# FeatureBaseDB/featurebase

Measured on NVIDIA H100. Metric: set_ops_per_sec, higher is better.
Workload: dtype u64/u16 integer

## Files before the change

### featurebase_b200/csrc/fbgpu.cu

```cuda
#include <cuda_runtime.h>
#include <dlfcn.h>
#include <fcntl.h>
#include <sys/mman.h>
#include <sys/stat.h>
#include <unistd.h>
#include <stdarg.h>
#include <stdio.h>
#include <string.h>

#include <algorithm>
#include <condition_variable>
#include <map>
#include <memory>
#include <mutex>
#include <shared_mutex>
#include <atomic>
#include <deque>
#include <functional>
#include <string>
#include <thread>
#include <unordered_map>
#include <vector>

#include "../../include/fbgpu.h"
// ... 793 lines not shown
    c->meta_dirty = true; c->tables_valid = false; c->dev_tables_valid = false;
    return commit_locked(c);
}

extern "C" int fbgpu_commit(fbgpu_ctx* c) try {
    if (!c) return fail(FBGPU_E_INVALID, "null ctx");
    std::unique_lock<std::shared_mutex> lk(c->store_mu);
    if (!c->inspect_only && c->dead_arena >= (256ull << 20) && c->dead_arena * 2 >= c->uploaded + c->staging.len) return compact_locked(c);
    return commit_locked(c);
} FBGPU_CATCH

extern "C" int fbgpu_compact(fbgpu_ctx* c) try {
    if (!c) return fail(FBGPU_E_INVALID, "null ctx");
    std::unique_lock<std::shared_mutex> lk(c->store_mu);
    return compact_locked(c);
} FBGPU_CATCH
static int lock_committed(fbgpu_ctx* c, std::shared_lock<std::shared_mutex>& lk) {
    if (c->inspect_only) return fail(FBGPU_E_CUDA, "this context was created with FBGPU_DEVICE_NONE: it holds no device and answers no query");
    for (;;) {
        lk = std::shared_lock<std::shared_mutex>(c->store_mu);
        if (!c->meta_dirty && c->staging.empty()) return 0;
        lk.unlock();
        int rc = fbgpu_commit(c); if (rc) return rc;
    }
}

extern "C" int fbgpu_get_stats(fbgpu_ctx* c, fbgpu_stats* out) try {
    if (!c || !out) return fail(FBGPU_E_INVALID, "null argument");
    std::shared_lock<std::shared_mutex> lk(c->store_mu);
    *out = c->stats;
    return 0;
} FBGPU_CATCH

static int compile_program(fbgpu_ctx* c, uint32_t index, const fbgpu_op* ops, int32_t n_ops, std::vector<DevOp>& out, int& depth) {
    Error err;
    ViewLookup lookup = [c, index](uint32_t field, uint32_t view) { return view_id_locked(c, ViewKey{ index, field, view }, false); };
    int rc = compile(ops, n_ops, lookup, out, depth, err);
    if (rc) return fail(rc, "%s", err.msg);
#ifndef FBGPU_WP_LEGACY_LOOP
    expand_push_row(out);
#endif
    return 0;
}

static void bump(fbgpu_ctx* c, uint64_t launches, float ms) {
    std::lock_guard<std::mutex> lk(c->cnt_mu);
    c->counters.kernel_launches += launches; c->counters.queries++; c->counters.last_query_gpu_ms = ms;
}

static int allreduce_u64(fbgpu_ctx* c, Workspace* w, void* dptr, size_t n) {
    if (!c->comm) return 0;
    std::lock_guard<std::mutex> lk(c->coll_mu);
    int r = g_nccl.AllReduce(dptr, dptr, n, kNcclUint64, kNcclSum, c->comm, w->stream);
    if (r != 0) return fail(FBGPU_E_COMM, "ncclAllReduce failed: %s", g_nccl.GetErrorString ? g_nccl.GetErrorString(r) : "?");
    return 0;
}

static std::vector<int2> find_batches(const std::vector<DevOp>& prog);
static int upload_inputs(Workspace* w, const std::vector<DevOp>& prog, const uint64_t* shards, int64_t n_shards, const DevOp** d_prog, const uint64_t** d_shards) {
    std::vector<int2> batches = find_batches(prog);
    size_t pb = prog.size() * sizeof(DevOp), sb = (size_t)n_shards * 8, bb = batches.size() * sizeof(int2), tot = pb + sb + bb;
    if (w->h_in.ensure(tot + 16)) return FBGPU_E_NOMEM;
    if (w->d_in.ensure(pb + sb + 16)) return FBGPU_E_NOMEM;
    if (w->d_aux.ensure(bb + 16)) return FBGPU_E_NOMEM;
    if (pb) memcpy(w->h_in.p, prog.data(), pb);
    if (sb) memcpy((uint8_t*)w->h_in.p + pb, shards, sb);
    if (bb) memcpy((uint8_t*)w->h_in.p + pb + sb, batches.data(), bb);
    if (pb + sb) CUDA_TRY(cudaMemcpyAsync(w->d_in.p, w->h_in.p, pb + sb, cudaMemcpyHostToDevice, w->stream));
    if (bb) CUDA_TRY(cudaMemcpyAsync(w->d_aux.p, (uint8_t*)w->h_in.p + pb + sb, bb, cudaMemcpyHostToDevice, w->stream));
    *d_prog = (const DevOp*)w->d_in.p; *d_shards = (const uint64_t*)((uint8_t*)w->d_in.p + pb);
    return 0;
}

static std::vector<int2> find_batches(const std::vector<DevOp>& prog) {
    std::vector<int2> b;
    for (size_t k = 0; k < prog.size();) {
        uint8_t o = prog[k].op;
        if (o == D_OR_ROW || o == D_ANDNOT_ROW || o == D_XOR_ROW) { size_t e = k + 1; while (e < prog.size() && prog[e].op == o) e++; b.push_back(make_int2((int)k, (int)e)); k = e; }
        else k++;
    }
    return b;
}

static int launch_eval(fbgpu_ctx* c, Workspace* w, const std::vector<DevOp>& prog, const DevOp* d_prog, int depth, const uint64_t* d_shards, long long n_units, EvalOut out) {
    if (n_units <= 0) return 0;
    const int n_ops = (int)prog.size();
    std::vector<int2> batches = find_batches(prog);
    size_t staged_rows = 0; for (auto& b : batches) staged_rows += (size_t)(b.y - b.x);
    if (!out.info && n_ops <= kWpMaxOps && depth <= kWpMaxDepth && !getenv("FBGPU_NO_WORDPAR")) {
        uint64_t arr = 0, other = 0, striped = 0;
        for (const DevOp& o : prog) if (o.op >= D_PUSH_ROW && o.op <= D_ORANDNOT_ROW && o.op != D_PUSH_EMPTY && o.fv < c->view_arr.size()) { arr += c->view_arr[o.fv]; other += c->view_other[o.fv]; striped += c->view_striped[o.fv]; }
        if (striped == 0 && ((other > 0 && arr * 8 <= other) || getenv("FBGPU_FORCE_WORDPAR") != nullptr)) {
            long long blocks = n_units * kWpBlocksPerUnit;
            long long grid = std::min<long long>(blocks, (long long)c->sm_count * std::max(FBGPU_WP_MIN_BLOCKS, 8) * 2);
            eval_wordpar_kernel<<<(unsigned)grid, kWpThreads, 0, w->stream>>>(store_ref(c), d_prog, n_ops, d_shards, n_units, out);
            CUDA_TRY(cudaGetLastError());
            return 0;
        }
    }
    const bool staged = getenv("FBGPU_STAGED") && n_ops <= kStagedMaxOps && staged_rows >= 4;
    const int2* d_batches = reinterpret_cast<const int2*>(w->d_aux.p);
    if (staged) {
        int ctas = 2;
        if (const char* e = getenv("FBGPU_STAGE_CTAS")) ctas = std::max(1, std::min(4, atoi(e)));
        const size_t per_cta = 233472 / ctas - 1024 - 5888;
        size_t stack = (size_t)(depth + 1) * 8192;
        if (stack + 2 * 8192 <= per_cta) {
            uint32_t stg = (uint32_t)(((per_cta - stack) / 2) & ~size_t(127));
            long long grid = std::min<long long>(n_units, (long long)c->sm_count * ctas);
            size_t smem = stack + 2 * (size_t)stg;
            eval_staged_kernel<<<(unsigned)grid, kEvalThreads, smem, w->stream>>>(store_ref(c), d_prog, n_ops, depth, d_batches, (int)batches.size(), stg, d_shards, n_units, out);
            CUDA_TRY(cudaGetLastError());
            return 0;
        }
    }
    size_t smem = (size_t)(depth + 1) * 8192;
    int per_sm = std::max(1, (int)std::min<size_t>(std::min(FBGPU_EVAL_MIN_BLOCKS, 2048 / kEvalThreads), (227 * 1024) / (smem + 3 * 1024 + 512)));
    long long grid = std::min<long long>(n_units, (long long)c->sm_count * per_sm);
    eval_kernel<<<(unsigned)grid, kEvalThreads, smem, w->stream>>>(store_ref(c), d_prog, n_ops, depth, d_batches, (int)batches.size(), d_shards, n_units, out);
    CUDA_TRY(cudaGetLastError());
    return 0;
}

static bool contiguous_shards(const uint64_t* shards, int64_t n) {
    for (int64_t i = 1; i < n; i++) if (shards[i] != shards[0] + (uint64_t)i) return false;
    return n > 0;
}

static int count_impl(fbgpu_ctx* c, uint32_t index, const fbgpu_op* ops, int32_t n_ops, const uint64_t* shards, int64_t n_shards,
                      uint64_t* out_total, uint64_t* out_per_shard, bool collective) {
    if (!c || !out_total || n_shards < 0 || (n_shards && !shards)) return fail(FBGPU_E_INVALID, "null argument");
    USE_DEVICE(c);
    std::shared_lock<std::shared_mutex> lk;
    int rc = lock_committed(c, lk); if (rc) return rc;
    std::vector<DevOp> prog; int depth = 1;
    rc = compile_program(c, index, ops, n_ops, prog, depth); if (rc) return rc;
    WsLease lease(c); Workspace* w = lease.w;
    const DevOp* d_prog; const uint64_t* d_shards;
    rc = upload_inputs(w, prog, shards, n_shards, &d_prog, &d_shards); if (rc) return rc;
    const size_t nper = out_per_shard ? (size_t)n_shards : 0, nc = 1 + nper + 3;
    if (w->d_counts.ensure(nc * 8)) return FBGPU_E_NOMEM;
    if (w->h_out.ensure(nc * 8)) return FBGPU_E_NOMEM;
    CUDA_TRY(cudaMemsetAsync(w->d_counts.p, 0, nc * 8, w->stream));
    unsigned long long* d_total = (unsigned long long*)w->d_counts.p;
    unsigned long long* d_per = out_per_shard ? d_total + 1 : nullptr;
    long long n_units = (long long)n_shards * kSlotsPerRow;
    std::unique_lock<std::mutex> coll_lk(c->coll_mu, std::defer_lock);
    FuseReduce fr{};
    coll_lk.lock();
    const bool p2p = c->p2p && collective;
    if (!p2p) coll_lk.unlock();
    if (p2p) {
        fr.peers = (Mailbox* const*)c->d_peers.p; fr.ticket = (unsigned int*)(d_total + 1 + nper); fr.result = d_total + 1 + nper + 1;
        fr.error = (unsigned int*)(d_total + 1 + nper + 2);
        fr.epoch = ++c->epoch; fr.rank = c->rank; fr.n_ranks = c->n_ranks; fr.timeout_cycles = c->p2p_timeout_cycles;
    }
    CUDA_TRY(cudaEventRecord(w->ev0, w->stream));
    if (n_units > 0) {
        const DevOp* pa = nullptr; const DevOp* pb = nullptr;
        if (prog.size() == 2 && prog[0].op == D_PUSH_ROW && prog[1].op == D_AND_ROW) { pa = &prog[0]; pb = &prog[1]; }
        else if (prog.size() == 3 && prog[0].op == D_PUSH_EMPTY && prog[1].op == D_OR_ROW && prog[2].op == D_AND_ROW) { pa = &prog[1]; pb = &prog[2]; }
        if (pa && !getenv("FBGPU_NO_PAIR_KERNEL")) {
            long long grid = std::min<long long>((n_units + kPcWarps - 1) / kPcWarps, (long long)c->sm_count * c->pair_ctas_per_sm);
            c->counters_pair_launches++;
            pair_count_kernel<<<(unsigned)grid, kPcWarps * 32, kPcWarps * 8192, w->stream>>>(store_ref(c), pa->fv, pa->row, pb->fv, pb->row, nullptr, nullptr, n_units,
                contiguous_shards(shards, n_shards) ? nullptr : d_shards, n_shards ? shards[0] : 0, n_units, d_total, d_per, nullptr, fr);
            CUDA_TRY(cudaGetLastError());
        } else {
            EvalOut eo{ d_total, d_per, nullptr, nullptr, fr };
            rc = launch_eval(c, w, prog, d_prog, depth, d_shards, n_units, eo); if (rc) return rc;
        }
    } else if (p2p) {
        p2p_reduce_only_kernel<<<1, 1, 0, w->stream>>>(fr, d_total);
        CUDA_TRY(cudaGetLastError());
    }
    if (!p2p && collective) { rc = allreduce_u64(c, w, d_total, 1); if (rc) return rc; }
    CUDA_TRY(cudaEventRecord(w->ev1, w->stream));
    CUDA_TRY(cudaMemcpyAsync(w->h_out.p, w->d_counts.p, nc * 8, cudaMemcpyDeviceToHost, w->stream));
    CUDA_TRY(cudaStreamSynchronize(w->stream));
    if (p2p && ((uint64_t*)w->h_out.p)[1 + nper + 2] != 0) {
        lease.ok = true;
        return fail(FBGPU_E_COMM, "rank %d did not publish its count for exchange %llu in time (peer dead, or the ranks issued their collective queries in different orders); re-open with fbgpu_comm_p2p_open",
                    (int)((uint64_t*)w->h_out.p)[1 + nper + 2] - 1, (unsigned long long)fr.epoch);
    }
    *out_total = p2p ? ((uint64_t*)w->h_out.p)[1 + nper + 1] : ((uint64_t*)w->h_out.p)[0];
    if (out_per_shard) memcpy(out_per_shard, (uint64_t*)w->h_out.p + 1, (size_t)n_shards * 8);
    float ms = 0; cudaEventElapsedTime(&ms, w->ev0, w->ev1);
    bump(c, (n_units > 0 || p2p) ? 1 : 0, ms);
    lease.ok = true;
    return FBGPU_OK;
}
extern "C" int fbgpu_count(fbgpu_ctx* c, uint32_t index, const fbgpu_op* ops, int32_t n_ops, const uint64_t* shards, int64_t n_shards,
                           uint64_t* out_total, uint64_t* out_per_shard) try {
    return count_impl(c, index, ops, n_ops, shards, n_shards, out_total, out_per_shard, true);
} FBGPU_CATCH
static int fbgpu_count_local(fbgpu_ctx* c, uint32_t index, const fbgpu_op* ops, int32_t n_ops, const uint64_t* shards, int64_t n_shards, uint64_t* out_total) {
    return count_impl(c, index, ops, n_ops, shards, n_shards, out_total, nullptr, false);
}

extern "C" int fbgpu_row(fbgpu_ctx* c, uint32_t index, const fbgpu_op* ops, int32_t n_ops, const uint64_t* shards, int64_t n_shards,
                         uint8_t* out_buf, uint64_t out_cap, uint64_t* out_len, uint64_t* out_count) try {
    if (!c || !out_len || n_shards < 0 || (n_shards && !shards)) return fail(FBGPU_E_INVALID, "null argument");
    USE_DEVICE(c);
    std::shared_lock<std::shared_mutex> lk;
    int rc = lock_committed(c, lk); if (rc) return rc;
    std::vector<DevOp> prog; int depth = 1;
    rc = compile_program(c, index, ops, n_ops, prog, depth); if (rc) return rc;
    std::vector<uint64_t> sorted(shards, shards + n_shards);
    std::sort(sorted.begin(), sorted.end());
    sorted.erase(std::unique(sorted.begin(), sorted.end()), sorted.end());
    n_shards = (int64_t)sorted.size();
    WsLease lease(c); Workspace* w = lease.w;
    const DevOp* d_prog; const uint64_t* d_shards;
    rc = upload_inputs(w, prog, sorted.data(), n_shards, &d_prog, &d_shards); if (rc) return rc;
    long long n_units = (long long)n_shards * kSlotsPerRow;
    struct OutCont { uint64_t key; uint16_t typ; uint32_t n; uint64_t size; uint32_t batch; uint64_t src_off; };
    std::vector<OutCont> conts; std::vector<std::vector<uint8_t>> batch_bufs;
    const bool single_batch = n_units <= c->unit_batch;
    const uint8_t* single_src = nullptr;
    uint64_t total_count = 0; uint64_t launches = 0; float ms_total = 0;
    for (long long u0 = 0; u0 < n_units; u0 += c->unit_batch) {
        long long nu = std::min(c->unit_batch, n_units - u0);
        if (w->d_bitmaps.ensure((size_t)nu * 8192)) return FBGPU_E_NOMEM;
        if (w->d_info.ensure((size_t)nu * 8)) return FBGPU_E_NOMEM;
        if (w->h_out.ensure((size_t)nu * 8)) return FBGPU_E_NOMEM;
        EvalOut eo{ nullptr, nullptr, (uint4*)w->d_bitmaps.p, (uint2*)w->d_info.p, FuseReduce{} };
        CUDA_TRY(cudaEventRecord(w->ev0, w->stream));
        rc = launch_eval(c, w, prog, d_prog, depth, d_shards + u0 / kSlotsPerRow, nu, eo); if (rc) return rc;
        launches++;
        CUDA_TRY(cudaMemcpyAsync(w->h_out.p, w->d_info.p, (size_t)nu * 8, cudaMemcpyDeviceToHost, w->stream));
        CUDA_TRY(cudaStreamSynchronize(w->stream));
        std::vector<EmitUnit> emits; uint64_t off = 0; size_t first = conts.size();
        const uint2* info = (const uint2*)w->h_out.p;
        for (long long u = 0; u < nu; u++) {
            uint32_t N = info[u].x, runs = info[u].y;
            if (!N) continue;
            uint16_t typ = (runs <= 2048 && runs <= N / 2) ? kRun : (N < 4096 ? kArray : kBitmap);
            uint64_t size = typ == kRun ? 2 + 4ull * runs : typ == kArray ? 2ull * N : 8192;
            EmitUnit e{ off, (uint32_t)u, typ };
            emits.push_back(e);
            OutCont oc; oc.key = sorted[(u0 + u) / kSlotsPerRow] * kSlotsPerRow + (uint64_t)((u0 + u) % kSlotsPerRow); oc.typ = typ; oc.n = N; oc.size = size;
            oc.batch = (uint32_t)batch_bufs.size(); oc.src_off = off;
            conts.push_back(oc);
            off += (size + 15) & ~15ull;
            total_count += N;
        }
        if (emits.empty()) batch_bufs.emplace_back();
        if (!emits.empty()) {
            if (w->d_emit_units.ensure(emits.size() * sizeof(EmitUnit))) return FBGPU_E_NOMEM;
// ... 707 lines not shown
```

### featurebase_b200/csrc/kernels.cuh

```cuda
#pragma once
#include <cuda_runtime.h>
#include <stdint.h>
#include "fbgpu_types.h"
#include "bitaddr.h"
#include "wp_machine.h"
#include "resolve.h"

namespace fbgpu {

#ifndef FBGPU_EVAL_THREADS
#define FBGPU_EVAL_THREADS 256
#endif
#ifndef FBGPU_EVAL_MIN_BLOCKS
#define FBGPU_EVAL_MIN_BLOCKS 6
#endif
constexpr int kEvalThreads = FBGPU_EVAL_THREADS;
constexpr int kEvalU4PerThread = 512 / kEvalThreads;
constexpr int kEvalW64PerThread = 1024 / kEvalThreads;
constexpr int kResolveChunk = 128;

__device__ __forceinline__ uint4 ldg_nc(const uint4* p) {
    uint4 r;
    asm volatile("ld.global.nc.L1::no_allocate.v4.u32 {%0,%1,%2,%3}, [%4];" : "=r"(r.x), "=r"(r.y), "=r"(r.z), "=r"(r.w) : "l"(p));
    return r;
// ... 71 lines not shown
    for (int h = 0; h < kEvalU4PerThread; h++) {
        int i = threadIdx.x + h * kEvalThreads;
        uint4 x = ldg_nc(g + i);
        switch (kind) {
            case K_PUSH: top[i] = x; break;
            case K_OR: top[i] = or4(top[i], x); break;
            case K_AND: top[i] = and4(top[i], x); break;
            case K_ANDNOT: top[i] = andn4(top[i], x); break;
            case K_XOR: top[i] = xor4(top[i], x); break;
            case K_ORAND: below[i] = or4(below[i], and4(top[i], x)); break;
            default: below[i] = or4(below[i], andn4(top[i], x)); break;
        }
    }
}
__device__ __forceinline__ void bm_apply_smem(int kind, uint4* top, uint4* below, const uint4* s) {
#pragma unroll
    for (int h = 0; h < kEvalU4PerThread; h++) {
        int i = threadIdx.x + h * kEvalThreads;
        uint4 x = s[i];
        switch (kind) {
            case K_PUSH: top[i] = x; break;
            case K_OR: top[i] = or4(top[i], x); break;
            case K_AND: top[i] = and4(top[i], x); break;
            case K_ANDNOT: top[i] = andn4(top[i], x); break;
            case K_XOR: top[i] = xor4(top[i], x); break;
            case K_ORAND: below[i] = or4(below[i], and4(top[i], x)); break;
            default: below[i] = or4(below[i], andn4(top[i], x)); break;
        }
    }
}

template <int MODE>
__device__ __forceinline__ void smem_bit_op(uint32_t* bm, uint32_t v) {
    uint32_t addr = (uint32_t)__cvta_generic_to_shared(bm + (v >> 5));
    uint32_t m = 1u << (v & 31);
    if (MODE == 0) asm volatile("red.shared.or.b32 [%0], %1;" :: "r"(addr), "r"(m) : "memory");
    else if (MODE == 1) asm volatile("red.shared.and.b32 [%0], %1;" :: "r"(addr), "r"(~m) : "memory");
    else asm volatile("red.shared.xor.b32 [%0], %1;" :: "r"(addr), "r"(m) : "memory");
}
template <int MODE>
__device__ __forceinline__ void warp_bitmap_atomic(uint32_t* bm, const uint4* g, int lane) {
    for (int i = lane; i < 512; i += 32) {
        uint4 v = ldg_nc(g + i);
        uint32_t w[4] = { v.x, v.y, v.z, v.w };
#pragma unroll
        for (int q = 0; q < 4; q++) {
            if (MODE == 0) atomicOr(&bm[4 * i + q], w[q]); else if (MODE == 1) atomicAnd(&bm[4 * i + q], ~w[q]); else atomicXor(&bm[4 * i + q], w[q]);
        }
    }
}
template <int MODE>
__device__ __forceinline__ void smem_bit_op_at(uint32_t addr, uint32_t sh) {
    const uint32_t m = 1u << (sh & 31);
    if (MODE == 0) asm volatile("red.shared.or.b32 [%0], %1;" :: "r"(addr), "r"(m) : "memory");
    else if (MODE == 1) asm volatile("red.shared.and.b32 [%0], %1;" :: "r"(addr), "r"(~m) : "memory");
    else asm volatile("red.shared.xor.b32 [%0], %1;" :: "r"(addr), "r"(m) : "memory");
}
template <int MODE>
__device__ __forceinline__ void scatter_chunk_sb(smem_base_t sb, uint4 v, uint32_t base, uint32_t n) {
    uint32_t w[4] = { v.x, v.y, v.z, v.w };
    if (MODE != 2 || base + 8 <= n) {
#pragma unroll
        for (int q = 0; q < 4; q++) {
            smem_bit_op_at<MODE>(word_addr_lo(sb, w[q]), w[q]);
            smem_bit_op_at<MODE>(word_addr_hi(sb, w[q]), upper16(w[q]));
        }
    } else {
#pragma unroll
        for (int q = 0; q < 4; q++) {
            if (base + 2 * q < n) smem_bit_op_at<MODE>(word_addr_lo(sb, w[q]), w[q]);
            if (base + 2 * q + 1 < n) smem_bit_op_at<MODE>(word_addr_hi(sb, w[q]), w[q] >> 16);
        }
    }
}
template <int MODE>
__device__ __forceinline__ void scatter_chunk_unrolled(uint32_t* bm, uint4 v, uint32_t base, uint32_t n) {
    scatter_chunk_sb<MODE>(smem_base((uint32_t)__cvta_generic_to_shared(bm)), v, base, n);
}
static_assert(sizeof(Resolved) == 16, "batch_rows reads a Resolved with one 16-byte shared load");
#ifndef FBGPU_EVAL_DEEP
#define FBGPU_EVAL_DEEP 3
#endif
template <int MODE>
__device__ __forceinline__ void batch_rows(uint32_t* T32, const Resolved* res, int n) {
    const int lane = threadIdx.x & 31, wid = threadIdx.x >> 5;
    smem_base_t sb = smem_base((uint32_t)__cvta_generic_to_shared(T32));
    pin_base(sb);
    for (int j = wid; j < n; j += kEvalThreads / 32) {
        const uint4 raw = *reinterpret_cast<const uint4*>(res + j);
        const uint4* a4 = reinterpret_cast<const uint4*>(((unsigned long long)raw.y << 32) | raw.x);
        if (a4 == nullptr) continue;
        const uint32_t typ = raw.w & 0xffffu;
        if (typ == kArray) {
            const uint32_t card = raw.z, n8 = (card + 7) >> 3;
            uint4 v[FBGPU_EVAL_DEEP];
#pragma unroll
            for (int q = 0; q < FBGPU_EVAL_DEEP; q++) v[q] = ldg_nc(a4 + min((uint32_t)lane + 32u * q, n8 - 1u));
#pragma unroll
            for (int q = 0; q < FBGPU_EVAL_DEEP; q++) if (lane + 32 * q < n8) scatter_chunk_sb<MODE>(sb, v[q], (lane + 32 * q) * 8, card);
            for (uint32_t i = lane + 32 * FBGPU_EVAL_DEEP; i < n8; i += 32) scatter_chunk_sb<MODE>(sb, ldg_nc(a4 + i), i * 8, card);
        } else if (typ == kBitmap) warp_bitmap_atomic<MODE>(T32, a4, lane);
    }
}
constexpr int kMaxRanks = 16;
struct Mailbox { unsigned long long value[2][kMaxRanks]; unsigned long long flag[2][kMaxRanks]; };
struct FuseReduce {
    Mailbox* const* peers;
    unsigned int* ticket;
    unsigned long long* result;
    unsigned int* error;
    unsigned long long epoch;
    long long timeout_cycles;
    int rank, n_ranks;
};
__device__ __forceinline__ void fused_allreduce_tail(const FuseReduce& fr, unsigned long long* total, unsigned int n_callers) {
    if (fr.peers == nullptr) return;
    __threadfence();
    if (atomicAdd(fr.ticket, 1u) != n_callers - 1) return;
    __threadfence();
    const unsigned long long mine = *reinterpret_cast<volatile unsigned long long*>(total);
    const int par = (int)(fr.epoch & 1ull);
    for (int p = 0; p < fr.n_ranks; p++) *reinterpret_cast<volatile unsigned long long*>(&fr.peers[p]->value[par][fr.rank]) = mine;
    __threadfence_system();
    for (int p = 0; p < fr.n_ranks; p++) *reinterpret_cast<volatile unsigned long long*>(&fr.peers[p]->flag[par][fr.rank]) = fr.epoch;
    __threadfence_system();
    Mailbox* me = fr.peers[fr.rank];
    unsigned long long sum = 0;
    for (int q = 0; q < fr.n_ranks; q++) {
        const long long t0 = clock64();
        while (*reinterpret_cast<volatile unsigned long long*>(&me->flag[par][q]) != fr.epoch) {
            if (clock64() - t0 > fr.timeout_cycles) { *fr.error = 1u + (unsigned int)q; *fr.result = ~0ull; __threadfence_system(); return; }
        }
        __threadfence_system();
        sum += *reinterpret_cast<volatile unsigned long long*>(&me->value[par][q]);
    }
    *fr.result = sum;
}
__global__ void p2p_reduce_only_kernel(FuseReduce fr, unsigned long long* total) { fused_allreduce_tail(fr, total, 1u); }

struct EvalOut {
    unsigned long long* total;
    unsigned long long* per_shard;
    uint4* bitmaps;
    uint2* info;
    FuseReduce fr;
};

__global__ void __launch_bounds__(kEvalThreads, FBGPU_EVAL_MIN_BLOCKS)
eval_kernel(StoreRef st, const DevOp* __restrict__ prog, int n_ops, int depth,
            const int2* __restrict__ batches, int n_batches,
            const uint64_t* __restrict__ shards, long long n_units, EvalOut out) {
    extern __shared__ uint4 smem4[];
    __shared__ __align__(16) Resolved res[kResolveChunk];
    __shared__ uint32_t warp_tmp[kEvalThreads / 32];
    __shared__ uint32_t warp_tmp2[kEvalThreads / 32];
    const int tid = threadIdx.x, lane = tid & 31, wid = tid >> 5;
    unsigned long long cta_total = 0;

    for (long long unit = blockIdx.x; unit < n_units; unit += gridDim.x) {
        const uint64_t shard = shards[unit >> 4];
        const int slot = (int)(unit & 15);
        uint64_t map = 0xFEDCBA9876543210ull;
        int top = -1;
        auto phys = [&](int level) -> uint4* { return smem4 + (size_t)((map >> (4 * level)) & 15u) * 512; };
        auto swap_levels = [&](int a, int b) {
            uint64_t pa = (map >> (4 * a)) & 15u, pb = (map >> (4 * b)) & 15u;
            map &= ~((15ull << (4 * a)) | (15ull << (4 * b)));
            map |= (pb << (4 * a)) | (pa << (4 * b));
        };
        int cur_batch = 0;
        for (int base = 0; base < n_ops; base += kResolveChunk) {
            int chunk = min(kResolveChunk, n_ops - base);
            __syncthreads();
            bool is_run = false;
            if (tid < chunk) {
                DevOp op = prog[base + tid];
                Resolved r; r.ptr = nullptr; r.card = 0; r.typ = 0; r.cnt = 0;
                if (op.op >= D_PUSH_ROW && op.op <= D_ORANDNOT_ROW && op.op != D_PUSH_EMPTY) r = resolve(st, op.fv, shard, op.row, slot);
                res[tid] = r;
                is_run = r.ptr != nullptr && r.typ == kRun;
            }
            const int has_runs = __syncthreads_or(is_run);
            for (int k = 0; k < chunk; k++) {
                const uint8_t opc = prog[base + k].op;
                if (opc == D_PUSH_EMPTY) { top++; bm_zero(phys(top)); __syncthreads(); continue; }
                if (opc == D_SWAP) { swap_levels(top, top - 1); continue; }
                if (opc == D_POP) { top--; continue; }
                if (opc >= D_AND && opc <= D_XOR) {
                    int kind = opc == D_AND ? K_AND : opc == D_OR ? K_OR : opc == D_ANDNOT ? K_ANDNOT : K_XOR;
                    bm_apply_smem(kind, phys(top - 1), nullptr, phys(top));
                    top--; __syncthreads(); continue;
                }
                if (opc == D_OR_ROW || opc == D_ANDNOT_ROW || opc == D_XOR_ROW) {
                    while (cur_batch < n_batches && batches[cur_batch].y <= base + k) cur_batch++;
                    const int e = min(cur_batch < n_batches ? batches[cur_batch].y - base : k + 1, chunk);
                    uint4* T = phys(top);
                    uint32_t* T32 = reinterpret_cast<uint32_t*>(T);
                    if (opc == D_OR_ROW) batch_rows<0>(T32, res + k, e - k);
                    else if (opc == D_ANDNOT_ROW) batch_rows<1>(T32, res + k, e - k);
                    else batch_rows<2>(T32, res + k, e - k);
                    __syncthreads();
                    if (has_runs) for (int j = k; j < e; j++) {
                        const Resolved r = res[j];
                        if (r.ptr == nullptr || r.typ != kRun) continue;
                        uint4* S = phys(depth);
                        bm_expand_runs(S, reinterpret_cast<const uint16_t*>(r.ptr), r.cnt, warp_tmp);
                        bm_apply_smem(opc == D_OR_ROW ? K_OR : opc == D_ANDNOT_ROW ? K_ANDNOT : K_XOR, T, nullptr, S);
                        __syncthreads();
                    }
                    k = e - 1;
                    continue;
                }
                int kind = opc == D_PUSH_ROW ? K_PUSH : opc == D_OR_ROW ? K_OR : opc == D_AND_ROW ? K_AND : opc == D_ANDNOT_ROW ? K_ANDNOT
                         : opc == D_XOR_ROW ? K_XOR : opc == D_ORAND_ROW ? K_ORAND : K_ORANDNOT;
                const Resolved r = res[k];
                if (kind == K_PUSH) top++;
                uint4* T = phys(top);
                uint4* B = (kind == K_ORAND || kind == K_ORANDNOT) ? phys(top - 1) : nullptr;
                if (r.ptr == nullptr) {
                    if (kind == K_PUSH || kind == K_AND) bm_zero(T);
                    else if (kind == K_ORANDNOT) bm_apply_smem(K_OR, B, nullptr, T);
                    __syncthreads();
                } else if (r.typ == kBitmap) {
                    bm_apply_global(kind, T, B, reinterpret_cast<const uint4*>(r.ptr));
                    __syncthreads();
                } else if (r.typ == kArray) {
                    const uint16_t* arr = reinterpret_cast<const uint16_t*>(r.ptr);
                    uint32_t* T32 = reinterpret_cast<uint32_t*>(T);
                    if (kind == K_PUSH) { bm_zero(T); __syncthreads(); bm_scatter<0>(T32, arr, r.card); }
                    else if (kind == K_OR) bm_scatter<0>(T32, arr, r.card);
                    else if (kind == K_ANDNOT) bm_scatter<1>(T32, arr, r.card);
                    else if (kind == K_XOR) bm_scatter<2>(T32, arr, r.card);
                    else if (kind == K_ORAND) bm_filter_scatter(reinterpret_cast<uint32_t*>(B), T32, arr, r.card);
                    else if (kind == K_AND) {
                        uint4* S = phys(depth);
                        bm_zero(S); __syncthreads();
                        bm_filter_scatter(reinterpret_cast<uint32_t*>(S), T32, arr, r.card);
                        swap_levels(top, depth);
                    } else {
                        uint4* S = phys(depth);
                        bm_zero(S); __syncthreads();
                        bm_scatter<0>(reinterpret_cast<uint32_t*>(S), arr, r.card); __syncthreads();
                        bm_apply_smem(K_ORANDNOT, T, B, S);
                    }
                    __syncthreads();
                } else {
                    const uint16_t* runs = reinterpret_cast<const uint16_t*>(r.ptr);
                    if (kind == K_PUSH) bm_expand_runs(T, runs, r.cnt, warp_tmp);
                    else {
                        uint4* S = phys(depth);
                        bm_expand_runs(S, runs, r.cnt, warp_tmp);
                        bm_apply_smem(kind, T, B, S);
                        __syncthreads();
                    }
                }
            }
        }
        uint32_t cnt = 0, nruns = 0;
        if (top >= 0) {
            const uint4* R = phys(top);
            const uint64_t* R64 = reinterpret_cast<const uint64_t*>(R);
#pragma unroll
            for (int h = 0; h < kEvalU4PerThread; h++) {
                int i = tid + h * kEvalThreads;
                uint4 a = R[i];
                cnt += popc4(a);
                if (out.bitmaps) out.bitmaps[(size_t)unit * 512 + i] = a;
                if (out.info) {
#pragma unroll
                    for (int q = 0; q < 2; q++) {
                        int wi = 2 * i + q;
                        uint64_t v = R64[wi];
                        uint64_t prev = wi ? (R64[wi - 1] >> 63) : 0ull;
                        nruns += __popcll(v & ~((v << 1) | prev));
                    }
                }
            }
        } else if (out.bitmaps) {
#pragma unroll
            for (int h = 0; h < kEvalU4PerThread; h++) out.bitmaps[(size_t)unit * 512 + tid + h * kEvalThreads] = make_uint4(0, 0, 0, 0);
        }
        cnt = __reduce_add_sync(0xffffffffu, cnt);
        nruns = __reduce_add_sync(0xffffffffu, nruns);
        __syncthreads();
        if (lane == 0) { warp_tmp[wid] = cnt; warp_tmp2[wid] = nruns; }
        __syncthreads();
        if (tid == 0) {
            uint32_t c = 0, rr = 0;
#pragma unroll
            for (int k = 0; k < kEvalThreads / 32; k++) { c += warp_tmp[k]; rr += warp_tmp2[k]; }
            cta_total += c;
            if (out.per_shard && c) atomicAdd(&out.per_shard[unit >> 4], (unsigned long long)c);
            if (out.info) out.info[unit] = make_uint2(c, rr);
        }
    }
    if (tid == 0 && out.total) { if (cta_total) atomicAdd(out.total, cta_total); fused_allreduce_tail(out.fr, out.total, gridDim.x); }
}

constexpr int kStageOps = 32;
constexpr int kStagedMaxOps = 128;

struct SubBatch { int seq, b, o0, n; uint32_t total, pad; uint32_t off[kStageOps]; uint32_t bytes[kStageOps]; };

__device__ __forceinline__ uint32_t smem_u32(const void* p) { return (uint32_t)__cvta_generic_to_shared(p); }
__device__ __forceinline__ void mbar_init(uint64_t* bar, uint32_t count) { asm volatile("mbarrier.init.shared::cta.b64 [%0], %1;" :: "r"(smem_u32(bar)), "r"(count) : "memory"); }
__device__ __forceinline__ void mbar_expect_tx(uint64_t* bar, uint32_t bytes) { asm volatile("mbarrier.arrive.expect_tx.shared::cta.b64 _, [%0], %1;" :: "r"(smem_u32(bar)), "r"(bytes) : "memory"); }
__device__ __forceinline__ bool mbar_try_wait(uint64_t* bar, uint32_t parity) {
    uint32_t ok;
    asm volatile("{\n .reg .pred p;\n mbarrier.try_wait.parity.shared::cta.b64 p, [%1], %2;\n selp.u32 %0, 1, 0, p;\n}" : "=r"(ok) : "r"(smem_u32(bar)), "r"(parity) : "memory");
    return ok != 0;
}
__device__ __forceinline__ void tma_bulk_g2s(void* dst_smem, const void* src_gmem, uint32_t bytes, uint64_t* bar) {
    asm volatile("cp.async.bulk.shared::cluster.global.mbarrier::complete_tx::bytes [%0], [%1], %2, [%3];"
                 :: "r"(smem_u32(dst_smem)), "l"(src_gmem), "r"(bytes), "r"(smem_u32(bar)) : "memory");
}

template <int MODE>
__device__ __forceinline__ void stage_scatter(uint32_t* T32, const uint8_t* stage, const SubBatch& S, const Resolved* R) {
    const int tid = threadIdx.x, n = S.n;
    int G = kEvalThreads / max(n, 1);
    G = G >= 32 ? 32 : G <= 1 ? 1 : (1 << (31 - __clz(G)));
    const int groups = kEvalThreads / G, g = tid & (G - 1);
    for (int j = tid / G; j < n; j += groups) {
        const uint32_t sz = S.bytes[j];
        if (!sz) continue;
        const Resolved r = R[S.o0 + j];
        const uint4* src = reinterpret_cast<const uint4*>(stage + S.off[j]);
        if (r.typ == kArray) {
            const uint32_t n8 = sz >> 4;
            for (uint32_t i = g; i < n8; i += G) scatter_chunk_unrolled<MODE>(T32, src[i], i * 8, r.card);
        } else {
            for (int i = g; i < 512; i += G) {
                uint4 v = src[i];
                uint32_t w[4] = { v.x, v.y, v.z, v.w };
#pragma unroll
                for (int c = 0; c < 4; c++) {
                    if (!w[c]) continue;
                    uint32_t* dst = &T32[4 * i + c];
                    if (MODE == 0) atomicOr(dst, w[c]); else if (MODE == 1) atomicAnd(dst, ~w[c]); else atomicXor(dst, w[c]);
                }
            }
        }
    }
}

#ifndef FBGPU_STAGED_MIN_BLOCKS
#define FBGPU_STAGED_MIN_BLOCKS 2
#endif
__global__ void __launch_bounds__(kEvalThreads, FBGPU_STAGED_MIN_BLOCKS)
eval_staged_kernel(StoreRef st, const DevOp* __restrict__ prog, int n_ops, int depth,
                   const int2* __restrict__ batches, int n_batches, uint32_t stg_bytes,
                   const uint64_t* __restrict__ shards, long long n_units, EvalOut out) {
    extern __shared__ uint4 smem4[];
    __shared__ Resolved res2[2][kStagedMaxOps];
    __shared__ SubBatch sb[2];
    __shared__ __align__(8) uint64_t mbar[2];
    __shared__ int it_seq, it_b, it_o, s_ni;
    __shared__ uint32_t warp_tmp[kEvalThreads / 32], warp_tmp2[kEvalThreads / 32];
    const int tid = threadIdx.x, lane = tid & 31, wid = tid >> 5;
    uint8_t* stage0 = reinterpret_cast<uint8_t*>(smem4 + (size_t)(depth + 1) * 512);
    const long long n_seq = (n_units - blockIdx.x + gridDim.x - 1) / gridDim.x;
    if (n_seq <= 0) return;
    if (tid == 0) { mbar_init(&mbar[0], 1); mbar_init(&mbar[1], 1); it_seq = 0; it_b = 0; it_o = n_batches ? batches[0].x : 0; s_ni = 0; asm volatile("fence.mbarrier_init.release.cluster;" ::: "memory"); }
    int nc = 0;
    unsigned long long cta_total = 0;

    auto resolve_unit = [&](long long seq) {
        if (tid < n_ops) {
            const long long unit = blockIdx.x + seq * gridDim.x;
            DevOp op = prog[tid];
            Resolved r; r.ptr = nullptr; r.card = 0; r.typ = 0; r.cnt = 0;
            if (op.op >= D_PUSH_ROW && op.op <= D_ORANDNOT_ROW && op.op != D_PUSH_EMPTY) r = resolve(st, op.fv, shards[unit >> 4], op.row, (int)(unit & 15));
            res2[seq & 1][tid] = r;
        }
    };
    auto pump = [&](long long avail) {
        for (;;) {
            const int ni = s_ni;
            if (ni - nc >= 2) break;
// ... 1620 lines not shown
```

Measured before the change: 124.2 million.

## Add specialized union-count kernel for AND of OR-unions with prefetched resolves

Detects count programs shaped as an intersection of several OR-unions of rows (up to three sides) and routes them to a new kernel. The kernel scatters each operand directly into a per-side shared-memory bitmap and fuses the AND and popcount in one pass. It also double-buffers container resolution so the next unit's lookups overlap the current unit's scatter. The generic stack interpreter stays as the fallback. Run containers are handled on a slower serialized path, and a standalone HBM read microbenchmark is added.

```diff
diff --git a/bench_micro/hbm_read.cu b/bench_micro/hbm_read.cu
--- /dev/null
+++ b/bench_micro/hbm_read.cu
@@ -0,0 +1,61 @@
+#include <cstdio>
+#include <cstdint>
+#include <cstdlib>
+#include <cuda_runtime.h>
+#define CK(x) do { cudaError_t e = (x); if (e != cudaSuccess) { printf("CUDA error %s at %s:%d\n", cudaGetErrorString(e), __FILE__, __LINE__); return 1; } } while (0)
+
+__device__ __forceinline__ uint4 ldg_nc(const uint4* p) {
+    uint4 r;
+    asm volatile("ld.global.nc.L1::no_allocate.v4.u32 {%0,%1,%2,%3}, [%4];" : "=r"(r.x), "=r"(r.y), "=r"(r.z), "=r"(r.w) : "l"(p));
+    return r;
+}
+
+template <int DEPTH>
+__global__ void __launch_bounds__(256) read_kernel(const uint4* __restrict__ src, size_t n16, unsigned int* out) {
+    const size_t stride = (size_t)gridDim.x * blockDim.x;
+    uint32_t acc = 0;
+    size_t i = (size_t)blockIdx.x * blockDim.x + threadIdx.x;
+    for (; i + (DEPTH - 1) * stride < n16; i += DEPTH * stride) {
+        uint4 v[DEPTH];
+#pragma unroll
+        for (int d = 0; d < DEPTH; d++) v[d] = ldg_nc(src + i + d * stride);
+#pragma unroll
+        for (int d = 0; d < DEPTH; d++) acc ^= v[d].x ^ v[d].y ^ v[d].z ^ v[d].w;
+    }
+    for (; i < n16; i += stride) { const uint4 v = ldg_nc(src + i); acc ^= v.x ^ v.y ^ v.z ^ v.w; }
+    if (acc == 0x9e3779b9u) atomicAdd(out, 1u);
+}
+
+template <int DEPTH>
+static int run(const uint4* buf, size_t n16, unsigned int* out, int grid, int iters) {
+    read_kernel<DEPTH><<<grid, 256>>>(buf, n16, out);
+    CK(cudaDeviceSynchronize());
+    cudaEvent_t e0, e1; CK(cudaEventCreate(&e0)); CK(cudaEventCreate(&e1));
+    CK(cudaEventRecord(e0));
+    for (int it = 0; it < iters; it++) read_kernel<DEPTH><<<grid, 256>>>(buf, n16, out);
+    CK(cudaEventRecord(e1)); CK(cudaEventSynchronize(e1));
+    float ms; CK(cudaEventElapsedTime(&ms, e0, e1));
+    const double per = ms / iters, gbs = (double)n16 * 16 / (per * 1e-3) / 1e9;
+    printf("grid %6d x 256 thr, %d loads in flight / thread: %8.4f ms per pass  %7.1f GB/s\n", grid, DEPTH, per, gbs);
+    return 0;
+}
+
+int main(int argc, char** argv) {
+    const size_t bytes = (argc > 1 ? strtoull(argv[1], nullptr, 10) : 1536ull) << 20;
+    const size_t n16 = bytes / 16;
+    cudaDeviceProp p; CK(cudaGetDeviceProperties(&p, 0));
+    printf("device: %s, %d SMs, buffer %.3f GB\n", p.name, p.multiProcessorCount, bytes / 1e9);
+    uint4* buf; unsigned int* out;
+    CK(cudaMalloc(&buf, bytes)); CK(cudaMalloc(&out, 4));
+    CK(cudaMemset(buf, 0x5a, bytes)); CK(cudaMemset(out, 0, 4));
+    const int sms = p.multiProcessorCount, iters = 50;
+    for (int per_sm : { 2, 4, 8 }) {
+        if (run<2>(buf, n16, out, sms * per_sm, iters)) return 1;
+        if (run<4>(buf, n16, out, sms * per_sm, iters)) return 1;
+        if (run<8>(buf, n16, out, sms * per_sm, iters)) return 1;
+    }
+    fflush(stdout);
+    if (system("nvidia-smi --query-gpu=name,power.limit,clocks.sm,clocks.max.sm,clocks.mem --format=csv") != 0) printf("nvidia-smi query failed\n");
+    CK(cudaFree(buf)); CK(cudaFree(out));
+    return 0;
+}
diff --git a/featurebase_b200/csrc/fbgpu.cu b/featurebase_b200/csrc/fbgpu.cu
--- a/featurebase_b200/csrc/fbgpu.cu
+++ b/featurebase_b200/csrc/fbgpu.cu
@@ -899,21 +899,24 @@
     return b;
 }
 
+static bool use_wordpar(fbgpu_ctx* c, const std::vector<DevOp>& prog, int depth, bool row_result) {
+    if (row_result || (int)prog.size() > kWpMaxOps || depth > kWpMaxDepth || getenv("FBGPU_NO_WORDPAR")) return false;
+    uint64_t arr = 0, other = 0, striped = 0;
+    for (const DevOp& o : prog) if (o.op >= D_PUSH_ROW && o.op <= D_ORANDNOT_ROW && o.op != D_PUSH_EMPTY && o.fv < c->view_arr.size()) { arr += c->view_arr[o.fv]; other += c->view_other[o.fv]; striped += c->view_striped[o.fv]; }
+    return striped == 0 && ((other > 0 && arr * 8 <= other) || getenv("FBGPU_FORCE_WORDPAR") != nullptr);
+}
+
 static int launch_eval(fbgpu_ctx* c, Workspace* w, const std::vector<DevOp>& prog, const DevOp* d_prog, int depth, const uint64_t* d_shards, long long n_units, EvalOut out) {
     if (n_units <= 0) return 0;
     const int n_ops = (int)prog.size();
     std::vector<int2> batches = find_batches(prog);
     size_t staged_rows = 0; for (auto& b : batches) staged_rows += (size_t)(b.y - b.x);
-    if (!out.info && n_ops <= kWpMaxOps && depth <= kWpMaxDepth && !getenv("FBGPU_NO_WORDPAR")) {
-        uint64_t arr = 0, other = 0, striped = 0;
-        for (const DevOp& o : prog) if (o.op >= D_PUSH_ROW && o.op <= D_ORANDNOT_ROW && o.op != D_PUSH_EMPTY && o.fv < c->view_arr.size()) { arr += c->view_arr[o.fv]; other += c->view_other[o.fv]; striped += c->view_striped[o.fv]; }
-        if (striped == 0 && ((other > 0 && arr * 8 <= other) || getenv("FBGPU_FORCE_WORDPAR") != nullptr)) {
-            long long blocks = n_units * kWpBlocksPerUnit;
-            long long grid = std::min<long long>(blocks, (long long)c->sm_count * std::max(FBGPU_WP_MIN_BLOCKS, 8) * 2);
-            eval_wordpar_kernel<<<(unsigned)grid, kWpThreads, 0, w->stream>>>(store_ref(c), d_prog, n_ops, d_shards, n_units, out);
-            CUDA_TRY(cudaGetLastError());
-            return 0;
-        }
+    if (use_wordpar(c, prog, depth, out.info != nullptr)) {
+        long long blocks = n_units * kWpBlocksPerUnit;
+        long long grid = std::min<long long>(blocks, (long long)c->sm_count * std::max(FBGPU_WP_MIN_BLOCKS, 8) * 2);
+        eval_wordpar_kernel<<<(unsigned)grid, kWpThreads, 0, w->stream>>>(store_ref(c), d_prog, n_ops, d_shards, n_units, out);
+        CUDA_TRY(cudaGetLastError());
+        return 0;
     }
     const bool staged = getenv("FBGPU_STAGED") && n_ops <= kStagedMaxOps && staged_rows >= 4;
     const int2* d_batches = reinterpret_cast<const int2*>(w->d_aux.p);
@@ -944,6 +947,19 @@
     return n > 0;
 }
 
+static bool union_count_operands(const std::vector<DevOp>& prog, std::vector<DevOp>& opnds, int& n_sides) {
+    opnds.clear(); n_sides = 0;
+    for (size_t k = 0; k < prog.size();) {
+        if (prog[k].op != D_PUSH_EMPTY || n_sides == kUcMaxSides) return false;
+        size_t e = k + 1;
+        for (; e < prog.size() && prog[e].op == D_OR_ROW; e++) { DevOp o = prog[e]; o.pad[0] = (uint8_t)n_sides; opnds.push_back(o); }
+        if (e == k + 1) return false;
+        if (n_sides > 0) { if (e == prog.size() || prog[e].op != D_AND) return false; e++; }
+        n_sides++; k = e;
+    }
+    return n_sides >= 2 && opnds.size() <= (size_t)kUcMaxOps;
+}
+
 static int count_impl(fbgpu_ctx* c, uint32_t index, const fbgpu_op* ops, int32_t n_ops, const uint64_t* shards, int64_t n_shards,
                       uint64_t* out_total, uint64_t* out_per_shard, bool collective) {
     if (!c || !out_total || n_shards < 0 || (n_shards && !shards)) return fail(FBGPU_E_INVALID, "null argument");
@@ -952,9 +968,11 @@
     int rc = lock_committed(c, lk); if (rc) return rc;
     std::vector<DevOp> prog; int depth = 1;
     rc = compile_program(c, index, ops, n_ops, prog, depth); if (rc) return rc;
+    std::vector<DevOp> opnds; int n_sides = 0;
+    const bool union_count = union_count_operands(prog, opnds, n_sides) && !getenv("FBGPU_NO_UNION_COUNT_KERNEL") && !use_wordpar(c, prog, depth, false);
     WsLease lease(c); Workspace* w = lease.w;
     const DevOp* d_prog; const uint64_t* d_shards;
-    rc = upload_inputs(w, prog, shards, n_shards, &d_prog, &d_shards); if (rc) return rc;
+    rc = upload_inputs(w, union_count ? opnds : prog, shards, n_shards, &d_prog, &d_shards); if (rc) return rc;
     const size_t nper = out_per_shard ? (size_t)n_shards : 0, nc = 1 + nper + 3;
     if (w->d_counts.ensure(nc * 8)) return FBGPU_E_NOMEM;
     if (w->h_out.ensure(nc * 8)) return FBGPU_E_NOMEM;
@@ -982,6 +1000,12 @@
             c->counters_pair_launches++;
             pair_count_kernel<<<(unsigned)grid, kPcWarps * 32, kPcWarps * 8192, w->stream>>>(store_ref(c), pa->fv, pa->row, pb->fv, pb->row, nullptr, nullptr, n_units,
                 contiguous_shards(shards, n_shards) ? nullptr : d_shards, n_shards ? shards[0] : 0, n_units, d_total, d_per, nullptr, fr);
+            CUDA_TRY(cudaGetLastError());
+        } else if (union_count) {
+            const size_t smem = (size_t)(n_sides + 1) * 8192;
+            const int per_sm = std::max(1, (int)std::min<size_t>(FBGPU_UC_MIN_BLOCKS, (227 * 1024) / (smem + 9 * 1024)));
+            const long long grid = std::min<long long>(n_units, (long long)c->sm_count * per_sm);
+            union_count_kernel<<<(unsigned)grid, kEvalThreads, smem, w->stream>>>(store_ref(c), d_prog, (int)opnds.size(), n_sides, d_shards, n_units, d_total, d_per, fr);
             CUDA_TRY(cudaGetLastError());
         } else {
             EvalOut eo{ d_total, d_per, nullptr, nullptr, fr };
diff --git a/featurebase_b200/csrc/kernels.cuh b/featurebase_b200/csrc/kernels.cuh
--- a/featurebase_b200/csrc/kernels.cuh
+++ b/featurebase_b200/csrc/kernels.cuh
@@ -177,6 +177,16 @@
 #define FBGPU_EVAL_DEEP 3
 #endif
 template <int MODE>
+__device__ __forceinline__ void warp_array_scatter(smem_base_t sb, const uint4* a4, uint32_t card, int lane) {
+    const uint32_t n8 = (card + 7) >> 3;
+    uint4 v[FBGPU_EVAL_DEEP];
+#pragma unroll
+    for (int q = 0; q < FBGPU_EVAL_DEEP; q++) v[q] = ldg_nc(a4 + min((uint32_t)lane + 32u * q, n8 - 1u));
+#pragma unroll
+    for (int q = 0; q < FBGPU_EVAL_DEEP; q++) if (lane + 32 * q < n8) scatter_chunk_sb<MODE>(sb, v[q], (lane + 32 * q) * 8, card);
+    for (uint32_t i = lane + 32 * FBGPU_EVAL_DEEP; i < n8; i += 32) scatter_chunk_sb<MODE>(sb, ldg_nc(a4 + i), i * 8, card);
+}
+template <int MODE>
 __device__ __forceinline__ void batch_rows(uint32_t* T32, const Resolved* res, int n) {
     const int lane = threadIdx.x & 31, wid = threadIdx.x >> 5;
     smem_base_t sb = smem_base((uint32_t)__cvta_generic_to_shared(T32));
@@ -186,15 +196,8 @@
         const uint4* a4 = reinterpret_cast<const uint4*>(((unsigned long long)raw.y << 32) | raw.x);
         if (a4 == nullptr) continue;
         const uint32_t typ = raw.w & 0xffffu;
-        if (typ == kArray) {
-            const uint32_t card = raw.z, n8 = (card + 7) >> 3;
-            uint4 v[FBGPU_EVAL_DEEP];
-#pragma unroll
-            for (int q = 0; q < FBGPU_EVAL_DEEP; q++) v[q] = ldg_nc(a4 + min((uint32_t)lane + 32u * q, n8 - 1u));
-#pragma unroll
-            for (int q = 0; q < FBGPU_EVAL_DEEP; q++) if (lane + 32 * q < n8) scatter_chunk_sb<MODE>(sb, v[q], (lane + 32 * q) * 8, card);
-            for (uint32_t i = lane + 32 * FBGPU_EVAL_DEEP; i < n8; i += 32) scatter_chunk_sb<MODE>(sb, ldg_nc(a4 + i), i * 8, card);
-        } else if (typ == kBitmap) warp_bitmap_atomic<MODE>(T32, a4, lane);
+        if (typ == kArray) warp_array_scatter<MODE>(sb, a4, raw.z, lane);
+        else if (typ == kBitmap) warp_bitmap_atomic<MODE>(T32, a4, lane);
     }
 }
 constexpr int kMaxRanks = 16;
@@ -390,6 +393,84 @@
         }
     }
     if (tid == 0 && out.total) { if (cta_total) atomicAdd(out.total, cta_total); fused_allreduce_tail(out.fr, out.total, gridDim.x); }
+}
+
+constexpr int kUcMaxOps = kEvalThreads;
+constexpr int kUcMaxSides = 3;
+#ifndef FBGPU_UC_MIN_BLOCKS
+#define FBGPU_UC_MIN_BLOCKS 6
+#endif
+
+__global__ void __launch_bounds__(kEvalThreads, FBGPU_UC_MIN_BLOCKS)
+union_count_kernel(StoreRef st, const DevOp* __restrict__ opnds, int n_opnds, int n_sides,
+                   const uint64_t* __restrict__ shards, long long n_units, unsigned long long* total, unsigned long long* per_shard, FuseReduce fr) {
+    extern __shared__ uint4 smem4[];
+    __shared__ __align__(16) Resolved res[2][kUcMaxOps];
+    __shared__ uint32_t warp_cnt[kEvalThreads / 32];
+    __shared__ uint32_t warp_tmp[kEvalThreads / 32];
+    __shared__ unsigned long long s_total;
+    const int tid = threadIdx.x, lane = tid & 31, wid = tid >> 5;
+    const smem_base_t sb0 = smem_base((uint32_t)__cvta_generic_to_shared(smem4));
+    auto resolve_into = [&](Resolved* R, long long unit) {
+        if (tid >= n_opnds) return;
+        const DevOp op = opnds[tid];
+        Resolved r = resolve(st, op.fv, shards[unit >> 4], op.row, (int)(unit & 15));
+        if (r.typ != kRun) r.cnt = op.pad[0];
+        R[tid] = r;
+    };
+    auto add_unit_count = [&](long long unit) {
+        uint32_t c = 0;
+#pragma unroll
+        for (int k = 0; k < kEvalThreads / 32; k++) c += warp_cnt[k];
+        s_total += c;
+        if (per_shard && c) atomicAdd(&per_shard[unit >> 4], (unsigned long long)c);
+    };
+    if (tid == 0) s_total = 0;
+    for (int s = 0; s <= n_sides; s++) bm_zero(smem4 + s * 512);
+    if (blockIdx.x < n_units) resolve_into(res[0], blockIdx.x);
+    int buf = 0;
+    for (long long unit = blockIdx.x; unit < n_units; unit += gridDim.x, buf ^= 1) {
+        __syncthreads();
+        if (tid == 0 && unit != blockIdx.x) add_unit_count(unit - gridDim.x);
+        const Resolved* R = res[buf];
+        bool saw_run = false;
+        for (int j = wid; j < n_opnds; j += kEvalThreads / 32) {
+            const uint4 raw = *reinterpret_cast<const uint4*>(R + j);
+            const uint4* a4 = reinterpret_cast<const uint4*>(((unsigned long long)raw.y << 32) | raw.x);
+            if (a4 == nullptr) continue;
+            const uint32_t typ = raw.w & 0xffffu, side = raw.w >> 16;
+            if (typ == kArray) warp_array_scatter<0>(sb0 + side * 8192u, a4, raw.z, lane);
+            else if (typ == kBitmap) warp_bitmap_atomic<0>(reinterpret_cast<uint32_t*>(smem4 + side * 512), a4, lane);
+            else saw_run = true;
+        }
+        if (unit + gridDim.x < n_units) resolve_into(res[buf ^ 1], unit + gridDim.x);
+        if (__syncthreads_or(saw_run)) {
+            uint4* S = smem4 + n_sides * 512;
+            for (int j = 0; j < n_opnds; j++) {
+                const Resolved r = R[j];
+                if (r.ptr == nullptr || r.typ != kRun) continue;
+                bm_expand_runs(S, reinterpret_cast<const uint16_t*>(r.ptr), r.cnt, warp_tmp);
+                bm_apply_smem(K_OR, smem4 + (uint32_t)opnds[j].pad[0] * 512, nullptr, S);
+                __syncthreads();
+            }
+        }
+        uint32_t cnt = 0;
+#pragma unroll
+        for (int h = 0; h < kEvalU4PerThread; h++) {
+            const int i = tid + h * kEvalThreads;
+            uint4 a = smem4[i];
+            smem4[i] = make_uint4(0, 0, 0, 0);
+            for (int s = 1; s < n_sides; s++) { a = and4(a, smem4[s * 512 + i]); smem4[s * 512 + i] = make_uint4(0, 0, 0, 0); }
+            cnt += popc4(a);
+        }
+        cnt = __reduce_add_sync(0xffffffffu, cnt);
+        if (lane == 0) warp_cnt[wid] = cnt;
+    }
+    __syncthreads();
+    if (tid == 0) {
+        if (blockIdx.x < n_units) add_unit_count(blockIdx.x + (n_units - 1 - blockIdx.x) / gridDim.x * gridDim.x);
+        if (total) { if (s_total) atomicAdd(total, s_total); fused_allreduce_tail(fr, total, gridDim.x); }
+    }
 }
 
 constexpr int kStageOps = 32;
```

After: 126.5 million, median of 6. +1.8%, better.

## Fuse final binary op into popcount and track pre-zeroed smem bitmaps

Applied to the files above, without the earlier changes.

When only counts are requested and the program ends with a stack binary op, that last op is folded into the popcount pass instead of writing a result bitmap and re-reading it. The fused pass also zeroes both operand buffers and marks them clean, so a later PUSH_EMPTY on a clean buffer skips its zero fill and barrier. Clean bits are cleared whenever a buffer may be dirtied. A standalone HBM read-bandwidth microbenchmark is also added. The clean-tracking is fragile: any write path that misses clearing its bit would leave stale data.

```diff
diff --git a/bench_micro/hbm_read.cu b/bench_micro/hbm_read.cu
--- /dev/null
+++ b/bench_micro/hbm_read.cu
@@ -0,0 +1,57 @@
+#include <cstdio>
+#include <cstdint>
+#include <cuda_runtime.h>
+#define CK(x) do { cudaError_t e = (x); if (e != cudaSuccess) { printf("CUDA error %s at %s:%d\n", cudaGetErrorString(e), __FILE__, __LINE__); return 1; } } while (0)
+
+__device__ __forceinline__ uint4 ldg_nc(const uint4* p) {
+    uint4 r;
+    asm volatile("ld.global.nc.L1::no_allocate.v4.u32 {%0,%1,%2,%3}, [%4];" : "=r"(r.x), "=r"(r.y), "=r"(r.z), "=r"(r.w) : "l"(p));
+    return r;
+}
+template <int UNROLL>
+__global__ void __launch_bounds__(512) read_kernel(const uint4* __restrict__ p, size_t n4, uint32_t* out) {
+    const size_t stride = (size_t)gridDim.x * blockDim.x;
+    uint32_t acc = 0;
+    size_t i = (size_t)blockIdx.x * blockDim.x + threadIdx.x;
+    for (; i + (UNROLL - 1) * stride < n4; i += UNROLL * stride) {
+        uint4 v[UNROLL];
+#pragma unroll
+        for (int u = 0; u < UNROLL; u++) v[u] = ldg_nc(p + i + u * stride);
+#pragma unroll
+        for (int u = 0; u < UNROLL; u++) acc ^= v[u].x ^ v[u].y ^ v[u].z ^ v[u].w;
+    }
+    for (; i < n4; i += stride) { uint4 v = ldg_nc(p + i); acc ^= v.x ^ v.y ^ v.z ^ v.w; }
+    if (acc == 0x9e3779b1u) out[0] = acc;
+}
+template <int UNROLL>
+int run(const uint4* p, size_t n4, uint32_t* out, int sms, int blocks_per_sm, int threads) {
+    const int grid = sms * blocks_per_sm;
+    read_kernel<UNROLL><<<grid, threads>>>(p, n4, out); CK(cudaDeviceSynchronize());
+    cudaEvent_t e0, e1; CK(cudaEventCreate(&e0)); CK(cudaEventCreate(&e1));
+    const int reps = 20;
+    CK(cudaEventRecord(e0));
+    for (int r = 0; r < reps; r++) read_kernel<UNROLL><<<grid, threads>>>(p, n4, out);
+    CK(cudaEventRecord(e1)); CK(cudaEventSynchronize(e1));
+    float ms; CK(cudaEventElapsedTime(&ms, e0, e1));
+    const double bytes = (double)n4 * 16 * reps;
+    printf("unroll %d  %4d CTAs x %3d threads  %8.3f ms/pass  %7.1f GB/s\n", UNROLL, grid, threads, ms / reps, bytes / (ms * 1e-3) / 1e9);
+    CK(cudaEventDestroy(e0)); CK(cudaEventDestroy(e1));
+    return 0;
+}
+int main() {
+    int dev = 0, sms, mhz_max;
+    cudaDeviceProp prop; CK(cudaGetDeviceProperties(&prop, dev));
+    CK(cudaDeviceGetAttribute(&sms, cudaDevAttrMultiProcessorCount, dev));
+    CK(cudaDeviceGetAttribute(&mhz_max, cudaDevAttrClockRate, dev));
+    const size_t bytes = 4ull << 30, n4 = bytes / 16;
+    printf("%s, %d SMs, max SM clock %d MHz, buffer %.2f GB\n", prop.name, sms, mhz_max / 1000, bytes / 1e9);
+    uint4* p; uint32_t* out;
+    CK(cudaMalloc(&p, bytes)); CK(cudaMalloc(&out, 4));
+    CK(cudaMemset(p, 0x5a, bytes));
+    if (run<1>(p, n4, out, sms, 4, 512)) return 1;
+    if (run<4>(p, n4, out, sms, 4, 512)) return 1;
+    if (run<8>(p, n4, out, sms, 4, 512)) return 1;
+    if (run<4>(p, n4, out, sms, 8, 256)) return 1;
+    CK(cudaFree(p)); CK(cudaFree(out));
+    return 0;
+}
diff --git a/featurebase_b200/csrc/kernels.cuh b/featurebase_b200/csrc/kernels.cuh
--- a/featurebase_b200/csrc/kernels.cuh
+++ b/featurebase_b200/csrc/kernels.cuh
@@ -251,21 +251,26 @@
     __shared__ uint32_t warp_tmp2[kEvalThreads / 32];
     const int tid = threadIdx.x, lane = tid & 31, wid = tid >> 5;
     unsigned long long cta_total = 0;
+    const uint8_t last_op = n_ops > 0 ? prog[n_ops - 1].op : 0;
+    const bool fused_count = !out.bitmaps && !out.info && last_op >= D_AND && last_op <= D_XOR;
+    const int n_main = fused_count ? n_ops - 1 : n_ops;
+    uint32_t clean = 0;
 
     for (long long unit = blockIdx.x; unit < n_units; unit += gridDim.x) {
         const uint64_t shard = shards[unit >> 4];
         const int slot = (int)(unit & 15);
         uint64_t map = 0xFEDCBA9876543210ull;
         int top = -1;
-        auto phys = [&](int level) -> uint4* { return smem4 + (size_t)((map >> (4 * level)) & 15u) * 512; };
+        auto phys_idx = [&](int level) -> uint32_t { return (uint32_t)(map >> (4 * level)) & 15u; };
+        auto phys = [&](int level) -> uint4* { return smem4 + (size_t)phys_idx(level) * 512; };
         auto swap_levels = [&](int a, int b) {
             uint64_t pa = (map >> (4 * a)) & 15u, pb = (map >> (4 * b)) & 15u;
             map &= ~((15ull << (4 * a)) | (15ull << (4 * b)));
             map |= (pb << (4 * a)) | (pa << (4 * b));
         };
         int cur_batch = 0;
-        for (int base = 0; base < n_ops; base += kResolveChunk) {
-            int chunk = min(kResolveChunk, n_ops - base);
+        for (int base = 0; base < n_main; base += kResolveChunk) {
+            int chunk = min(kResolveChunk, n_main - base);
             __syncthreads();
             bool is_run = false;
             if (tid < chunk) {
@@ -278,7 +283,13 @@
             const int has_runs = __syncthreads_or(is_run);
             for (int k = 0; k < chunk; k++) {
                 const uint8_t opc = prog[base + k].op;
-                if (opc == D_PUSH_EMPTY) { top++; bm_zero(phys(top)); __syncthreads(); continue; }
+                if (opc == D_PUSH_EMPTY) {
+                    top++;
+                    const uint32_t bit = 1u << phys_idx(top);
+                    if (!(clean & bit)) { bm_zero(phys(top)); __syncthreads(); }
+                    clean &= ~bit;
+                    continue;
+                }
                 if (opc == D_SWAP) { swap_levels(top, top - 1); continue; }
                 if (opc == D_POP) { top--; continue; }
                 if (opc >= D_AND && opc <= D_XOR) {
@@ -299,6 +310,7 @@
                         const Resolved r = res[j];
                         if (r.ptr == nullptr || r.typ != kRun) continue;
                         uint4* S = phys(depth);
+                        clean &= ~(1u << phys_idx(depth));
                         bm_expand_runs(S, reinterpret_cast<const uint16_t*>(r.ptr), r.cnt, warp_tmp);
                         bm_apply_smem(opc == D_OR_ROW ? K_OR : opc == D_ANDNOT_ROW ? K_ANDNOT : K_XOR, T, nullptr, S);
                         __syncthreads();
@@ -306,6 +318,7 @@
                     k = e - 1;
                     continue;
                 }
+                clean = 0;
                 int kind = opc == D_PUSH_ROW ? K_PUSH : opc == D_OR_ROW ? K_OR : opc == D_AND_ROW ? K_AND : opc == D_ANDNOT_ROW ? K_ANDNOT
                          : opc == D_XOR_ROW ? K_XOR : opc == D_ORAND_ROW ? K_ORAND : K_ORANDNOT;
                 const Resolved r = res[k];
@@ -352,7 +365,19 @@
             }
         }
         uint32_t cnt = 0, nruns = 0;
-        if (top >= 0) {
+        if (fused_count) {
+            uint4* A = phys(top - 1);
+            uint4* B = phys(top);
+#pragma unroll
+            for (int h = 0; h < kEvalU4PerThread; h++) {
+                const int i = tid + h * kEvalThreads;
+                const uint4 a = A[i], b = B[i];
+                cnt += popc4(last_op == D_AND ? and4(a, b) : last_op == D_OR ? or4(a, b) : last_op == D_ANDNOT ? andn4(a, b) : xor4(a, b));
+                A[i] = make_uint4(0, 0, 0, 0);
+                B[i] = make_uint4(0, 0, 0, 0);
+            }
+            clean |= (1u << phys_idx(top - 1)) | (1u << phys_idx(top));
+        } else if (top >= 0) {
             const uint4* R = phys(top);
             const uint64_t* R64 = reinterpret_cast<const uint64_t*>(R);
 #pragma unroll
```

Result: faster. 121.7 million before, 124.3 million after, median of 6 (+2.2%).
